# miha-stopar/Plonky3-mobile

Hardware: AMD Instinct MI355X
Metric: fib_air proofs/sec (higher is better)
Workload: dtype u32 (BabyBear Montgomery, 31-bit modular)

## Files before the change

plonky3-mobile_amd/csrc/mmcs.hip:

```cpp
#include <algorithm>

#include "common.h"
#include "mmcs.h"
#include "poseidon2.hip.h"
#include "poseidon2_coop.hip.h"
#include "poseidon2_f64.hip.h"
#include "poseidon2_q4.hip.h"
#include "keccak.hip.h"

namespace p3 {

constexpr int MAX_CLASS_MATS = 16;

struct RowSet {
    const uint32_t* ptr[MAX_CLASS_MATS];
    uint32_t width[MAX_CLASS_MATS];
    uint32_t stride[MAX_CLASS_MATS];
    uint32_t count;
    uint32_t total;
};

__device__ __forceinline__ void load_digest(const uint32_t* p, uint32_t* out8) {
    const uint4* q = reinterpret_cast<const uint4*>(p);
    uint4 a = q[0], b = q[1];
// ... 82 lines not shown
        if (act) {
#pragma unroll
            for (int k = 0; k < 8; k++) lds[tid * 8 + k] = s[k];
            store_digest(out + tid * 8, s);
        }
        __syncthreads();
        out += (size_t)half * 8;
    }
}


__global__ void __launch_bounds__(256) leaf_hash_f64_kernel(const uint32_t* mat, uint32_t width, uint64_t n_rows, uint32_t* digests) {
    if (gridDim.x <= 512u) P3_LATENCY_BOUND_KERNEL();
    uint64_t r = (uint64_t)blockIdx.x * blockDim.x + threadIdx.x;
    if (r >= n_rows) return;
    double s[16];
#pragma unroll
    for (int i = 0; i < 16; i++) s[i] = 0.0;
    const uint32_t* row = mat + r * width;
    for (uint32_t k = 0; k < width; k += 8) {
#pragma unroll
        for (int i = 0; i < 8; i++)
            if (k + i < width) s[i] = p2f::load_elem(row[k + i]);
        p2f::permute(s);
        if (k + 8 < width) {
#pragma unroll
            for (int i = 0; i < 16; i++) s[i] = p2f::reduce(s[i]);
        }
    }
    uint32_t d[8];
    const p2f::MagicRegs smk = p2f::magic_regs();
#pragma unroll
    for (int i = 0; i < 8; i++) d[i] = p2f::store_elem(s[i], smk);
    store_digest(digests + r * 8, d);
}
__global__ void __launch_bounds__(256) compress_layer_q4_kernel(const uint32_t* prev, uint32_t* next, uint64_t n_out, uint32_t prio) {
    if (prio) P3_LATENCY_BOUND_KERNEL();
    const uint32_t q = threadIdx.x & 3u;
    const uint64_t i = ((uint64_t)blockIdx.x * blockDim.x + threadIdx.x) >> 2;
    const bool act = i < n_out;
    const p2q::LaneConsts lc = p2q::lane_consts(q);
    double s[4] = {0.0, 0.0, 0.0, 0.0};
    if (act) {
        const uint4 w = *reinterpret_cast<const uint4*>(prev + i * 16 + 4 * q);
        s[0] = p2f::load_elem(w.x); s[1] = p2f::load_elem(w.y); s[2] = p2f::load_elem(w.z); s[3] = p2f::load_elem(w.w);
    }
    p2q::permute(s, lc, q == 0);
    if (act && q < 2) {
        const p2f::MagicRegs smk = p2f::magic_regs();
        *reinterpret_cast<uint4*>(next + i * 8 + 4 * q) =
            make_uint4(p2f::store_elem(s[0], smk), p2f::store_elem(s[1], smk), p2f::store_elem(s[2], smk), p2f::store_elem(s[3], smk));
    }
}
__global__ void __launch_bounds__(256) leaf_hash_q4_kernel(const uint32_t* mat, uint32_t width, uint64_t n_rows, uint32_t* digests, uint32_t prio) {
    if (prio) P3_LATENCY_BOUND_KERNEL();
    const uint32_t q = threadIdx.x & 3u;
    const uint64_t r = ((uint64_t)blockIdx.x * blockDim.x + threadIdx.x) >> 2;
    const bool act = r < n_rows;
    const p2q::LaneConsts lc = p2q::lane_consts(q);
    double s[4] = {0.0, 0.0, 0.0, 0.0};
    const uint32_t* row = mat + (act ? r : 0) * width;
    for (uint32_t k = 0; k < width; k += 8) {
        if (act && q < 2) {
#pragma unroll
            for (uint32_t i = 0; i < 4; i++)
                if (k + 4 * q + i < width) s[i] = p2f::load_elem(row[k + 4 * q + i]);
        }
        p2q::permute(s, lc, q == 0);
        if (k + 8 < width) {
#pragma unroll
            for (int i = 0; i < 4; i++) s[i] = p2f::reduce(s[i]);
        }
    }
    if (act && q < 2) {
        const p2f::MagicRegs smk = p2f::magic_regs();
        *reinterpret_cast<uint4*>(digests + r * 8 + 4 * q) =
            make_uint4(p2f::store_elem(s[0], smk), p2f::store_elem(s[1], smk), p2f::store_elem(s[2], smk), p2f::store_elem(s[3], smk));
    }
}
constexpr uint32_t LEAF_WIDE_CHUNK = 32, LEAF_WIDE_STRIDE = 36;
__global__ void __launch_bounds__(256) leaf_hash_f64_wide_kernel(const uint32_t* mat, uint32_t width, uint64_t n_rows, uint32_t* digests) {
    __shared__ __attribute__((aligned(16))) uint32_t tile[256 * LEAF_WIDE_STRIDE];
    const uint32_t tid = threadIdx.x, col = tid & 31u, rsub = tid >> 5;
    const uint64_t r0 = (uint64_t)blockIdx.x * 256u, r = r0 + tid;
    double s[16];
#pragma unroll
    for (int i = 0; i < 16; i++) s[i] = 0.0;
    uint32_t pre[32];
    auto fetch = [&](uint32_t c0) {
#pragma unroll
        for (uint32_t i = 0; i < 32; i++) {
            const uint64_t row = r0 + rsub + 8u * i;
            pre[i] = (row < n_rows && c0 + col < width) ? mat[row * width + c0 + col] : 0u;
        }
    };
    fetch(0);
    for (uint32_t c0 = 0; c0 < width; c0 += LEAF_WIDE_CHUNK) {
        __syncthreads();
#pragma unroll
        for (uint32_t i = 0; i < 32; i++) tile[(rsub + 8u * i) * LEAF_WIDE_STRIDE + col] = pre[i];
        __syncthreads();
        if (c0 + LEAF_WIDE_CHUNK < width) fetch(c0 + LEAF_WIDE_CHUNK);
        const uint4* mine = reinterpret_cast<const uint4*>(tile + tid * LEAF_WIDE_STRIDE);
#pragma unroll 1
        for (uint32_t k = 0; k < LEAF_WIDE_CHUNK && c0 + k < width; k += 8) {
            const uint4 a = mine[k / 4], b = mine[k / 4 + 1];
            const uint32_t w[8] = {a.x, a.y, a.z, a.w, b.x, b.y, b.z, b.w};
#pragma unroll
            for (int i = 0; i < 8; i++)
                if (c0 + k + i < width) s[i] = p2f::load_elem(w[i]);
            p2f::permute(s);
            if (c0 + k + 8 < width) {
#pragma unroll
                for (int i = 0; i < 16; i++) s[i] = p2f::reduce(s[i]);
            }
        }
    }
    if (r >= n_rows) return;
    uint32_t d[8];
    const p2f::MagicRegs smk = p2f::magic_regs();
#pragma unroll
    for (int i = 0; i < 8; i++) d[i] = p2f::store_elem(s[i], smk);
    store_digest(digests + r * 8, d);
}
__global__ void __launch_bounds__(256) leaf_hash_f64_rowset_kernel(RowSet rs, uint64_t n_rows, uint32_t* digests) {
    if (gridDim.x <= 512u) P3_LATENCY_BOUND_KERNEL();
    uint64_t r = (uint64_t)blockIdx.x * blockDim.x + threadIdx.x;
    if (r >= n_rows) return;
    double s[16];
#pragma unroll
    for (int i = 0; i < 16; i++) s[i] = 0.0;
    uint32_t m = 0, off = 0;
    for (uint32_t k = 0; k < rs.total; k += 8) {
#pragma unroll
        for (int i = 0; i < 8; i++) {
            if (k + i < rs.total) {
                while (off >= rs.width[m]) { m++; off = 0; }
                s[i] = p2f::load_elem(rs.ptr[m][r * rs.stride[m] + off]);
                off++;
            }
        }
        p2f::permute(s);
        if (k + 8 < rs.total) {
#pragma unroll
            for (int i = 0; i < 16; i++) s[i] = p2f::reduce(s[i]);
        }
    }
    uint32_t d[8];
    const p2f::MagicRegs smk = p2f::magic_regs();
#pragma unroll
    for (int i = 0; i < 8; i++) d[i] = p2f::store_elem(s[i], smk);
    store_digest(digests + r * 8, d);
}
__global__ void __launch_bounds__(256) compress_layer_f64_kernel(const uint32_t* prev, uint32_t* next, uint64_t n_out) {
    if (gridDim.x <= 512u) P3_LATENCY_BOUND_KERNEL();
    uint64_t i = (uint64_t)blockIdx.x * blockDim.x + threadIdx.x;
    if (i >= n_out) return;
    uint32_t w[16];
    load_digest(prev + i * 16, w);
    load_digest(prev + i * 16 + 8, w + 8);
    double s[16];
#pragma unroll
    for (int k = 0; k < 16; k++) s[k] = p2f::load_elem(w[k]);
    p2f::permute(s);
    uint32_t d[8];
    const p2f::MagicRegs smk = p2f::magic_regs();
#pragma unroll
    for (int k = 0; k < 8; k++) d[k] = p2f::store_elem(s[k], smk);
    store_digest(next + i * 8, d);
}

__global__ void __launch_bounds__(256) compress_coop_kernel(const uint32_t* prev, uint32_t* next, uint32_t n_out) {
    P3_LATENCY_BOUND_KERNEL();
    const uint32_t lane16 = threadIdx.x & 15;
    const p2c::LaneConst lc = p2c::lane_constants(lane16);
    uint32_t i = (blockIdx.x * blockDim.x + threadIdx.x) >> 4;
    bool act = i < n_out;
    uint32_t v = act ? prev[(size_t)i * 16 + lane16] : 0u;
    v = p2c::permute(v, lc);
    if (act && lane16 < 8) next[(size_t)i * 8 + lane16] = v;
}
__global__ void __launch_bounds__(256) leaf_coop_kernel(const uint32_t* mat, uint32_t width, uint32_t n_rows, uint32_t* digests) {
    P3_LATENCY_BOUND_KERNEL();
    const uint32_t lane16 = threadIdx.x & 15;
    const p2c::LaneConst lc = p2c::lane_constants(lane16);
    uint32_t r = (blockIdx.x * blockDim.x + threadIdx.x) >> 4;
    bool act = r < n_rows;
    uint32_t v = 0;
    for (uint32_t k = 0; k < width; k += 8) {
        if (act && lane16 < 8 && k + lane16 < width) v = mat[(size_t)r * width + k + lane16];
        v = p2c::permute(v, lc);
    }
    if (act && lane16 < 8) digests[(size_t)r * 8 + lane16] = v;
}
__global__ void __launch_bounds__(1024) tree_levels_coop_kernel(uint32_t* layer_in, uint32_t n_in, uint32_t chunk, uint32_t levels,
                                                                uint32_t* root_copy) {
    P3_LATENCY_BOUND_KERNEL();
    __shared__ uint32_t lds[128 * 8];
    const uint32_t tid = threadIdx.x, lane16 = tid & 15, grp = tid >> 4;
    const p2c::LaneConst lc = p2c::lane_constants(lane16);
    const uint32_t* src = layer_in + (size_t)blockIdx.x * chunk * 8;
    for (uint32_t i = tid; i < chunk * 8; i += blockDim.x) lds[i] = src[i];
    __syncthreads();
    uint32_t* out = layer_in + (size_t)n_in * 8;
    uint32_t cur_n = n_in;
    for (uint32_t l = 0; l < levels; l++) {
        const uint32_t half = chunk >> (l + 1);
        const bool wave_active = ((tid >> 6) << 2) < half;
        uint32_t res = 0;
        if (wave_active) {
            uint32_t v = grp < half ? lds[grp * 16 + lane16] : 0u;
            res = p2c::permute(v, lc);
        }
        __syncthreads();
        if (grp < half && lane16 < 8) {
            lds[grp * 8 + lane16] = res;
            out[((size_t)blockIdx.x * half + grp) * 8 + lane16] = res;
            if (cur_n == 2 && root_copy) root_copy[lane16] = res;
        }
        __syncthreads();
        cur_n >>= 1;
        out += (size_t)cur_n * 8;
    }
}

__global__ void poseidon2_permute_kernel(uint32_t* states, uint64_t n) {
    uint64_t i = (uint64_t)blockIdx.x * blockDim.x + threadIdx.x;
    if (i >= n) return;
    uint32_t s[16];
    uint4* q = reinterpret_cast<uint4*>(states + i * 16);
#pragma unroll
    for (int k = 0; k < 4; k++) { uint4 v = q[k]; s[4 * k] = v.x; s[4 * k + 1] = v.y; s[4 * k + 2] = v.z; s[4 * k + 3] = v.w; }
    p2::permute(s);
#pragma unroll
    for (int k = 0; k < 4; k++) q[k] = make_uint4(s[4 * k], s[4 * k + 1], s[4 * k + 2], s[4 * k + 3]);
}


__global__ void poseidon2_permute_f64_kernel(uint32_t* states, uint64_t n) {
    uint64_t i = (uint64_t)blockIdx.x * blockDim.x + threadIdx.x;
    if (i >= n) return;
    double s[16];
    uint4* q = reinterpret_cast<uint4*>(states + i * 16);
#pragma unroll
    for (int k = 0; k < 4; k++) {
        uint4 v = q[k];
        s[4 * k] = p2f::load_elem(v.x); s[4 * k + 1] = p2f::load_elem(v.y); s[4 * k + 2] = p2f::load_elem(v.z); s[4 * k + 3] = p2f::load_elem(v.w);
    }
    p2f::permute(s);
#pragma unroll
    for (int k = 0; k < 4; k++)
        q[k] = make_uint4(p2f::store_elem(s[4 * k]), p2f::store_elem(s[4 * k + 1]), p2f::store_elem(s[4 * k + 2]), p2f::store_elem(s[4 * k + 3]));
}

__global__ void poseidon2_f64_probe_kernel(const double* in, uint32_t* out, uint64_t n, int mode) {
    uint64_t i = (uint64_t)blockIdx.x * blockDim.x + threadIdx.x;
    if (i >= n) return;
    double s[16];
#pragma unroll
    for (int k = 0; k < 16; k++) s[k] = in[i * 16 + k];
    if (mode == 0) p2f::permute(s);
    else if (mode == 1) p2f::internal_rounds(s, p2f::magic_regs());
    else {
#pragma unroll
        for (int k = 0; k < 16; k++) s[k] = p2f::reduce(s[k]);
    }
#pragma unroll
    for (int k = 0; k < 16; k++) out[i * 16 + k] = p2f::store_elem(s[k]);
}
__global__ void __launch_bounds__(256) poseidon2_q4_probe_kernel(const double* in, uint32_t* out, uint64_t n) {
    const uint32_t q = threadIdx.x & 3u;
    const uint64_t i = ((uint64_t)blockIdx.x * blockDim.x + threadIdx.x) >> 2;
    const bool act = i < n;
    const p2q::LaneConsts lc = p2q::lane_consts(q);
    double s[4] = {0.0, 0.0, 0.0, 0.0};
    if (act) {
#pragma unroll
        for (int k = 0; k < 4; k++) s[k] = in[i * 16 + 4 * q + k];
    }
    p2q::permute(s, lc, q == 0);
    if (act) {
#pragma unroll
        for (int k = 0; k < 4; k++) out[i * 16 + 4 * q + k] = p2f::store_elem(s[k]);
    }
}
int poseidon2_f64_probe(hipStream_t stream, const double* d_in, uint32_t* d_out, uint64_t n, int mode) {
    if (!n) return OK;
    if (mode == 3) hipLaunchKernelGGL(poseidon2_q4_probe_kernel, dim3((uint32_t)((n * 4 + 255) / 256)), dim3(256), 0, stream, d_in, d_out, n);
    else hipLaunchKernelGGL(poseidon2_f64_probe_kernel, dim3((uint32_t)((n + 255) / 256)), dim3(256), 0, stream, d_in, d_out, n, mode);
    P3_HIP(hipGetLastError());
    return OK;
}
__global__ void __launch_bounds__(256) poseidon2_permute_q4_kernel(uint32_t* states, uint64_t n) {
    const uint32_t q = threadIdx.x & 3u;
    const uint64_t i = ((uint64_t)blockIdx.x * blockDim.x + threadIdx.x) >> 2;
    const bool act = i < n;
    const p2q::LaneConsts lc = p2q::lane_consts(q);
    double s[4] = {0.0, 0.0, 0.0, 0.0};
    uint4* mine = reinterpret_cast<uint4*>(states + (act ? i : 0) * 16 + 4 * q);
    if (act) {
        const uint4 w = *mine;
        s[0] = p2f::load_elem(w.x); s[1] = p2f::load_elem(w.y); s[2] = p2f::load_elem(w.z); s[3] = p2f::load_elem(w.w);
    }
    p2q::permute(s, lc, q == 0);
    if (act) {
        const p2f::MagicRegs smk = p2f::magic_regs();
        *mine = make_uint4(p2f::store_elem(s[0], smk), p2f::store_elem(s[1], smk), p2f::store_elem(s[2], smk), p2f::store_elem(s[3], smk));
    }
}
__global__ void __launch_bounds__(256) poseidon2_permute_coop_kernel(uint32_t* states, uint64_t n) {
    const uint32_t lane16 = threadIdx.x & 15;
    const p2c::LaneConst lc = p2c::lane_constants(lane16);
    const uint64_t i = ((uint64_t)blockIdx.x * blockDim.x + threadIdx.x) >> 4;
    const bool act = i < n;
    uint32_t v = act ? states[i * 16 + lane16] : 0u;
    v = p2c::permute(v, lc);
    if (act) states[i * 16 + lane16] = v;
}
int poseidon2_permute_states_variant(hipStream_t stream, uint32_t* d_states, uint64_t n, int variant) {
    if (!n) return OK;
    if (variant == 3) hipLaunchKernelGGL(poseidon2_permute_coop_kernel, dim3((uint32_t)((n * 16 + 255) / 256)), dim3(256), 0, stream, d_states, n);
    else if (variant == 2) hipLaunchKernelGGL(poseidon2_permute_q4_kernel, dim3((uint32_t)((n * 4 + 255) / 256)), dim3(256), 0, stream, d_states, n);
    else if (variant == 1) hipLaunchKernelGGL(poseidon2_permute_f64_kernel, dim3((uint32_t)((n + 255) / 256)), dim3(256), 0, stream, d_states, n);
    else hipLaunchKernelGGL(poseidon2_permute_kernel, dim3((uint32_t)((n + 255) / 256)), dim3(256), 0, stream, d_states, n);
    P3_HIP(hipGetLastError());
    return OK;
}

int poseidon2_permute_states(hipStream_t stream, uint32_t* d_states, uint64_t n) {
    return poseidon2_permute_states_variant(stream, d_states, n, 1);
}

__device__ __forceinline__ uint32_t rowset_elem(const RowSet& rs, uint64_t r, uint32_t k, uint32_t& m, uint32_t& base) {
    while (k - base >= rs.width[m]) { base += rs.width[m]; m++; }
    return rs.ptr[m][r * rs.stride[m] + (k - base)];
}
__device__ __forceinline__ void keccak_sponge_row(const RowSet& rs, uint64_t r, uint64_t (&st)[25]) {
#pragma unroll
    for (int i = 0; i < 25; i++) st[i] = 0;
    const uint32_t n = rs.total, n64 = (n + 1) / 2;
    uint32_t m = 0, base = 0;
    for (uint32_t i = 0; i < n64; i += 17) {
#pragma unroll
        for (int k = 0; k < 17; k++) {
            const uint32_t e = 2 * (i + k);
            if (e < n) {
                uint64_t lo = rowset_elem(rs, r, e, m, base);
                uint64_t hi = e + 1 < n ? rowset_elem(rs, r, e + 1, m, base) : 0u;
                st[k] = lo | (hi << 32);
            }
        }
        if (i + 17 >= n64) kk::permute_digest(st);
        else kk::permute(st);
    }
}
__device__ __forceinline__ void store_digest64(uint32_t* p, const uint64_t (&st)[25]) {
    uint4* q = reinterpret_cast<uint4*>(p);
    q[0] = make_uint4((uint32_t)st[0], (uint32_t)(st[0] >> 32), (uint32_t)st[1], (uint32_t)(st[1] >> 32));
    q[1] = make_uint4((uint32_t)st[2], (uint32_t)(st[2] >> 32), (uint32_t)st[3], (uint32_t)(st[3] >> 32));
}
__global__ void __launch_bounds__(256) keccak_leaf_kernel(RowSet rs, uint64_t n_rows, uint32_t* digests) {
    if (gridDim.x <= 512u) P3_LATENCY_BOUND_KERNEL();
    uint64_t r = (uint64_t)blockIdx.x * blockDim.x + threadIdx.x;
    if (r >= n_rows) return;
    uint64_t st[25];
    keccak_sponge_row(rs, r, st);
    store_digest64(digests + r * 8, st);
}
template <int NP>
struct SaltedRows {
    const uint32_t* mat[NP];
    const uint32_t* salt[NP];
    uint32_t stride;
};
template <int W, int NP>
__global__ void __launch_bounds__(256) keccak_leaf_salted_kernel(SaltedRows<NP> a, uint64_t n_rows, uint32_t* digests) {
    static_assert((W == 4 || W == 6 || W == 8) && NP * (W + 4) <= 34, "one rate block");
    if (gridDim.x <= 512u) P3_LATENCY_BOUND_KERNEL();
    const uint64_t r = (uint64_t)blockIdx.x * blockDim.x + threadIdx.x;
    if (r >= n_rows) return;
    uint64_t st[25];
#pragma unroll
    for (int i = 0; i < 25; i++) st[i] = 0;
#pragma unroll
    for (int p = 0; p < NP; p++) {
        constexpr int L = (W + 4) / 2;
        const uint32_t* m = a.mat[p] + r * a.stride;
        if constexpr (W == 6) {
            const uint2* q = reinterpret_cast<const uint2*>(m);
#pragma unroll
            for (int k = 0; k < 3; k++) { const uint2 v = q[k]; st[p * L + k] = (uint64_t)v.x | ((uint64_t)v.y << 32); }
        } else {
// ... 539 lines not shown
```

plonky3-mobile_amd/csrc/poseidon2_f64.hip.h:

```cpp
#pragma once
#include "poseidon2.hip.h"

namespace p2f {

constexpr double PD = 2013265921.0;
constexpr double PINV = 1.0 / 2013265921.0;

__device__ __forceinline__ double mulmod(double a, double b) {
    double h = a * b;
    double l = __fma_rn(a, b, -h);
    double q = __builtin_rint(h * PINV);
    double r = __fma_rn(-q, PD, h);
    return r + l;
}
constexpr double PM1 = 2013265920.0;
__device__ __forceinline__ double mulmod_p(double a, double b, double aP) {
    double q = __builtin_rint(b * aP);
    double t = __fma_rn(a, b, -(q * PM1));
    return t - q;
}
__device__ __forceinline__ double reduce(double x) {
    return __fma_rn(-__builtin_rint(x * PINV), PD, x);
}
__device__ __forceinline__ double add_scaled_pow2(double tot, double x, double inv) {
    double xt = __fma_rn(x, inv, tot);
    double fr = __builtin_amdgcn_fract(xt);
    return __fma_rn(fr, -PD, xt);
}
constexpr double MAGIC = 6755399441055744.0;
constexpr double MAGIC_P = 6755399441055744.0 * 2013265921.0;
struct MagicRegs { double m, mp; };
__device__ __forceinline__ MagicRegs magic_regs() {
    MagicRegs r{MAGIC, MAGIC_P};
    asm volatile("" : "+v"(r.m), "+v"(r.mp));
    return r;
}
__device__ __forceinline__ double mulmod_m(double a, double b, double aP, const MagicRegs& k, double neg_pm1) {
    const double qb = __fma_rn(b, aP, k.m);
    const double c = __fma_rn(qb, neg_pm1, k.mp);
    const double t = __fma_rn(a, b, c);
    return t - qb;
}
__device__ __forceinline__ double sbox7(double x, const MagicRegs& k, double neg_pm1, double pinv) {
    const double xP = x * pinv;
    const double x2 = mulmod_m(x, x, xP, k, neg_pm1), x3 = mulmod_m(x, x2, xP, k, neg_pm1), x4 = mulmod_m(x, x3, xP, k, neg_pm1);
    return mulmod_m(x3, x4, x3 * pinv, k, neg_pm1);
}

struct ConstsF64 {
    double ext[8][16];
    double in[13];
    double k3, k15, i4, i8, i16, i256;
    double neg_pm1, pinv;
};
constexpr uint32_t c_from_monty(uint32_t m) {
    uint32_t t = m * bb::MU;
    uint64_t u = (uint64_t)t * bb::P;
    uint32_t uh = (uint32_t)(u >> 32);
    return uh ? bb::P - uh : 0;
}
constexpr uint64_t c_powmod(uint64_t b, uint64_t e) { uint64_t r = 1; b %= bb::P; while (e) { if (e & 1) r = r * b % bb::P; b = b * b % bb::P; e >>= 1; } return r; }
constexpr ConstsF64 make_consts() {
    ConstsF64 c{};
    for (int r = 0; r < 4; r++)
        for (int i = 0; i < 16; i++) {
            c.ext[r][i] = (double)c_from_monty(P3_RC16_EXT_INIT_MONTY[r][i]);
            c.ext[4 + r][i] = (double)c_from_monty(P3_RC16_EXT_FINAL_MONTY[r][i]);
        }
    for (int r = 0; r < 13; r++) c.in[r] = (double)c_from_monty(P3_RC16_INTERNAL_MONTY[r]);
    c.k3 = 3.0; c.k15 = 15.0; c.i4 = 0.25; c.i8 = 0.125; c.i16 = 0.0625; c.i256 = 0.00390625;
    c.neg_pm1 = -2013265920.0; c.pinv = 1.0 / 2013265921.0;
    return c;
}
static __device__ __constant__ ConstsF64 d_c = make_consts();

__device__ __forceinline__ void mat4(double& a, double& b, double& c, double& d) {
    double t01 = a + b, t23 = c + d, t0123 = t01 + t23;
    double t01123 = t0123 + b, t01233 = t0123 + d;
    double nd = __fma_rn(a, 2.0, t01233), nb = __fma_rn(c, 2.0, t01123);
    double na = t01123 + t01, nc = t01233 + t23;
    a = na; b = nb; c = nc; d = nd;
}
__device__ __forceinline__ void external_linear(double (&s)[16]) {
#pragma unroll
    for (int i = 0; i < 16; i += 4) mat4(s[i], s[i + 1], s[i + 2], s[i + 3]);
    double t[4];
#pragma unroll
    for (int k = 0; k < 4; k++) t[k] = (s[k] + s[k + 4]) + (s[k + 8] + s[k + 12]);
#pragma unroll
    for (int i = 0; i < 16; i++) s[i] += t[i & 3];
}

__device__ __forceinline__ void internal_rounds(double (&s)[16], const MagicRegs& mk) {
    const double npm1 = d_c.neg_pm1, pinv = d_c.pinv;
    const double k3 = d_c.k3, k15 = d_c.k15, i4 = d_c.i4, i8 = d_c.i8, i16 = d_c.i16, i256 = d_c.i256;
    auto internal_round = [&](int r) {
        s[0] = sbox7(s[0] + d_c.in[r], mk, npm1, pinv);
        double tot = ((s[0] + s[1]) + (s[2] + s[3])) + ((s[4] + s[5]) + (s[6] + s[7])) +
                     (((s[8] + s[9]) + (s[10] + s[11])) + ((s[12] + s[13]) + (s[14] + s[15])));
        tot = reduce(tot);
        s[0] = __fma_rn(s[0], -2.0, tot);
        s[1] = tot + s[1];
        s[2] = __fma_rn(s[2], 2.0, tot);
        s[3] = add_scaled_pow2(tot, s[3], 0.5);
        s[4] = __fma_rn(s[4], k3, tot);
        s[5] = __fma_rn(s[5], 4.0, tot);
        s[6] = add_scaled_pow2(tot, s[6], -0.5);
        s[7] = __fma_rn(s[7], -k3, tot);
        s[8] = __fma_rn(s[8], -4.0, tot);
        s[9] = add_scaled_pow2(tot, s[9], i256);
        s[10] = add_scaled_pow2(tot, s[10], i4);
        s[11] = add_scaled_pow2(tot, s[11], i8);
        s[12] = __fma_rn(s[12], -k15, tot);
        s[13] = add_scaled_pow2(tot, s[13], -i256);
        s[14] = add_scaled_pow2(tot, s[14], -i16);
        s[15] = __fma_rn(s[15], k15, tot);
    };
    auto fold_integer_lanes = [&]() {
        s[1] = reduce(s[1]); s[2] = reduce(s[2]); s[4] = reduce(s[4]); s[5] = reduce(s[5]);
        s[7] = reduce(s[7]); s[8] = reduce(s[8]); s[12] = reduce(s[12]); s[15] = reduce(s[15]);
    };
    _Pragma("clang loop unroll(disable)")
    for (int blk = 0; blk < 3; blk++) {
        _Pragma("clang loop unroll(disable)")
        for (int r = 0; r < 4; r++) internal_round(4 * blk + r);
        fold_integer_lanes();
    }
    internal_round(12);
    fold_integer_lanes();
}

__device__ __forceinline__ void permute(double (&s)[16]) {
    const MagicRegs mk = magic_regs();
    const double npm1 = d_c.neg_pm1, pinv = d_c.pinv;
    external_linear(s);
    _Pragma("clang loop unroll(disable)")
    for (int r = 0; r < 4; r++) {
#pragma unroll
        for (int i = 0; i < 16; i++) s[i] = sbox7(s[i] + d_c.ext[r][i], mk, npm1, pinv);
        external_linear(s);
    }
    internal_rounds(s, mk);
    _Pragma("clang loop unroll(disable)")
    for (int r = 4; r < 8; r++) {
#pragma unroll
        for (int i = 0; i < 16; i++) s[i] = sbox7(s[i] + d_c.ext[r][i], mk, npm1, pinv);
        external_linear(s);
    }
}

__device__ __forceinline__ double load_elem(uint32_t monty) { return (double)bb::from_monty(monty); }
constexpr double R_MOD_P = 268435454.0;
constexpr double R_MOD_P_OVER_P = 268435454.0 / 2013265921.0;
__device__ __forceinline__ uint32_t store_elem(double v, const MagicRegs& k) {
    const double r = mulmod_m(R_MOD_P, v, R_MOD_P_OVER_P, k, d_c.neg_pm1);
    const uint32_t w = (uint32_t)(int32_t)r;
    return min(w, w + bb::P);
}
__device__ __forceinline__ uint32_t store_elem(double v) { return store_elem(v, magic_regs()); }

}
```

plonky3-mobile_amd/csrc/prover.hip:

```cpp
#include <chrono>
#include <cstddef>
#include <deque>
#include <memory>
#include <cstring>

#include "bb31.hip.h"
#include "challenger.h"
#include "common.h"
#include "keccak.hip.h"
#include "mmcs.h"
#include "poseidon2.hip.h"
#include "poseidon2_f64.hip.h"
#include "prover.h"
#include "rng.h"
#include "rng_dev.hip.h"
#include "transcript.hip.h"

namespace p3 {

using bb::Ext;

__device__ __forceinline__ uint32_t tl(const TwoLevelTable& t, uint32_t e) {
    return bb::mul(t.lo[e & ((1u << t.T) - 1u)], t.hi[e >> t.T]);
}
// ... 70 lines not shown
    const DenConsts k0 = ds->k0, k1 = ds->k1;
    uint32_t t = blockIdx.x * blockDim.x + threadIdx.x;
    uint32_t j0 = t * DEN_CHUNK;
    if (j0 >= big) return;
    uint32_t a0[2 * DEN_CHUNK], e0[2 * DEN_CHUNK], e1[2 * DEN_CHUNK], nrm[2 * DEN_CHUNK], pre[2 * DEN_CHUNK];
#pragma unroll
    for (int k = 0; k < DEN_CHUNK; k++) {
        uint32_t x = bb::mul(gen, tl(roots, brev((j0 + k) & (big - 1), log_big)));
#pragma unroll
        for (int z = 0; z < 2; z++) {
            const DenConsts& c = z ? k1 : k0;
            const uint32_t a = bb::sub(c.z0, x);
            const uint32_t dd0 = bb::add(bb::sqr(a), c.k0), dd1 = bb::sub(bb::mul(c.k1, a), c.c1);
            a0[2 * k + z] = a; e0[2 * k + z] = dd0; e1[2 * k + z] = dd1;
            nrm[2 * k + z] = bb::sub(bb::sqr(dd0), bb::mul(bb::W_MONTY, bb::sqr(dd1)));
        }
    }
    uint32_t acc = bb::ONE;
#pragma unroll
    for (int k = 0; k < 2 * DEN_CHUNK; k++) { pre[k] = acc; acc = bb::mul(acc, nrm[k]); }
    uint32_t inv = bb::inv(acc);
#pragma unroll
    for (int k = 2 * DEN_CHUNK - 1; k >= 0; k--) {
        const uint32_t r = bb::mul(inv, pre[k]);
        inv = bb::mul(inv, nrm[k]);
        nrm[k] = r;
    }
#pragma unroll
    for (int k = 0; k < DEN_CHUNK; k++) {
        if (j0 + k >= big) break;
#pragma unroll
        for (int z = 0; z < 2; z++) {
            const DenConsts& c = z ? k1 : k0;
            const uint32_t i = 2 * k + z;
            const uint32_t f0 = bb::mul(e0[i], nrm[i]), f1 = bb::neg(bb::mul(e1[i], nrm[i]));
            Ext r;
            r.c[0] = bb::add(bb::mul(a0[i], f0), bb::mul(c.z2w, f1));
            r.c[2] = bb::add(bb::mul(a0[i], f1), bb::mul(c.z2, f0));
            r.c[1] = bb::neg(bb::add(bb::mul(c.z1, f0), bb::mul(c.z3w, f1)));
            r.c[3] = bb::neg(bb::add(bb::mul(c.z1, f1), bb::mul(c.z3, f0)));
            st_ext((z ? d1 : d0) + 4 * (size_t)(j0 + k), r);
        }
    }
}

constexpr int BARY_BLOCK = 256;
__global__ void __launch_bounds__(BARY_BLOCK) barycentric_kernel(TwoLevelTable roots, uint32_t n, uint32_t log_big,
                                                                 uint32_t gen, const uint2* lde_t, const uint4* lde_q,
                                                                 const uint32_t* d0, const uint32_t* d1,
                                                                 uint32_t* partials) {
    Ext acc[8];
#pragma unroll
    for (int k = 0; k < 8; k++) acc[k] = bb::ext_zero();
    const uint32_t step = gridDim.x * blockDim.x;
    for (uint32_t j = blockIdx.x * blockDim.x + threadIdx.x; j < n; j += 2 * step) {
        const bool two = j + step < n;
        const uint32_t j2 = two ? j + step : j;
        const uint32_t xa = bb::mul(gen, tl(roots, brev(j, log_big))), xb = two ? bb::mul(gen, tl(roots, brev(j2, log_big))) : 0u;
        const Ext e0a = bb::scale(ld_ext(d0 + 4 * (size_t)j), xa), e1a = bb::scale(ld_ext(d1 + 4 * (size_t)j), xa);
        const Ext e0b = bb::scale(ld_ext(d0 + 4 * (size_t)j2), xb), e1b = bb::scale(ld_ext(d1 + 4 * (size_t)j2), xb);
        const uint2 ta = lde_t[j], tb = lde_t[j2];
        const uint4 qa = lde_q[j], qb = lde_q[j2];
        auto fma2 = [](Ext& s, const Ext& ea, uint32_t va, const Ext& eb, uint32_t vb) {
#pragma unroll
            for (int c = 0; c < 4; c++) s.c[c] = bb::add(s.c[c], bb::dot2(ea.c[c], va, eb.c[c], vb));
        };
        fma2(acc[0], e0a, ta.x, e0b, tb.x);
        fma2(acc[1], e0a, ta.y, e0b, tb.y);
        fma2(acc[2], e1a, ta.x, e1b, tb.x);
        fma2(acc[3], e1a, ta.y, e1b, tb.y);
        fma2(acc[4], e0a, qa.x, e0b, qb.x);
        fma2(acc[5], e0a, qa.y, e0b, qb.y);
        fma2(acc[6], e0a, qa.z, e0b, qb.z);
        fma2(acc[7], e0a, qa.w, e0b, qb.w);
    }
    __shared__ uint32_t red[BARY_BLOCK / 64][32];
    const uint32_t lane = threadIdx.x & 63, wave = threadIdx.x >> 6;
#pragma unroll
    for (int k = 0; k < 8; k++)
#pragma unroll
        for (int c = 0; c < 4; c++) {
            uint32_t v = acc[k].c[c];
#pragma unroll
            for (int off = 32; off > 0; off >>= 1) v = bb::add(v, (uint32_t)__shfl_down((int)v, off, 64));
            if (lane == 0) red[wave][4 * k + c] = v;
        }
    __syncthreads();
    if (threadIdx.x < 32) {
        uint32_t v = 0;
#pragma unroll
        for (int w = 0; w < BARY_BLOCK / 64; w++) v = bb::add(v, red[w][threadIdx.x]);
        partials[blockIdx.x * 32 + threadIdx.x] = v;
    }
}

struct ReducedArgs {
    const uint2* lde_t;
    const uint4* lde_q;
    const uint32_t* d0;
    const uint32_t* d1;
    uint32_t* ro;
    const DevState* ds;
    uint32_t big;
};
__global__ void __launch_bounds__(256) reduced_openings_kernel(ReducedArgs a) {
    uint32_t j = blockIdx.x * blockDim.x + threadIdx.x;
    if (j >= a.big) return;
    const DevState* __restrict__ ds = a.ds;
    uint2 t = a.lde_t[j];
    uint4 q = a.lde_q[j];
    Ext u, w;
#pragma unroll
    for (int c = 0; c < 4; c++) {
        u.c[c] = bb::add(bb::add(bb::dot2(ds->alp[4].c[c], q.x, ds->alp[5].c[c], q.y), bb::dot2(ds->alp[6].c[c], q.z, ds->alp[7].c[c], q.w)),
                         bb::mul(ds->alp[1].c[c], t.y));
        w.c[c] = bb::dot2(ds->alp[2].c[c], t.x, ds->alp[3].c[c], t.y);
    }
    u.c[0] = bb::add(u.c[0], t.x);
    Ext e0 = ld_ext(a.d0 + 4 * (size_t)j), e1 = ld_ext(a.d1 + 4 * (size_t)j);
    Ext r = bb::add(bb::mul(bb::sub(ds->y02, u), e0), bb::mul(bb::sub(ds->y1, w), e1));
    st_ext(a.ro + 4 * (size_t)j, r);
}

__global__ void __launch_bounds__(256) fri_fold_kernel(TwoLevelTable inv_roots , const uint32_t* in,
                                                       uint32_t* out, uint32_t half, uint32_t log_half,
                                                       const DevState* __restrict__ ds, uint32_t round, uint32_t one_half) {
    if (gridDim.x <= 512u) P3_LATENCY_BOUND_KERNEL();
    uint32_t i = blockIdx.x * blockDim.x + threadIdx.x;
    if (i >= half) return;
    const Ext half_beta = ds->half_beta[round];
    Ext lo = ld_ext(in + 8 * (size_t)i), hi = ld_ext(in + 8 * (size_t)i + 4);
    uint32_t p = tl(inv_roots, brev(i, log_half));
    Ext s = bb::scale(bb::add(lo, hi), one_half);
    Ext d = bb::mul(bb::scale(half_beta, p), bb::sub(lo, hi));
    st_ext(out + 4 * (size_t)i, bb::add(s, d));
}

__global__ void __launch_bounds__(256) fri_fold_rollin_kernel(TwoLevelTable inv_roots , const uint32_t* in,
                                                              const uint32_t* __restrict__ ro, uint32_t* out, uint32_t half,
                                                              uint32_t log_half, const DevState* __restrict__ ds, uint32_t round,
                                                              uint32_t one_half) {
    if (gridDim.x <= 512u) P3_LATENCY_BOUND_KERNEL();
    uint32_t i = blockIdx.x * blockDim.x + threadIdx.x;
    if (i >= half) return;
    const Ext half_beta = ds->half_beta[round];
    const Ext beta2 = bb::sqr(bb::add(half_beta, half_beta));
    Ext lo = ld_ext(in + 8 * (size_t)i), hi = ld_ext(in + 8 * (size_t)i + 4), e = ld_ext(ro + 4 * (size_t)i);
    uint32_t p = tl(inv_roots, brev(i, log_half));
    Ext s = bb::scale(bb::add(lo, hi), one_half);
    Ext d = bb::mul(bb::scale(half_beta, p), bb::sub(lo, hi));
    st_ext(out + 4 * (size_t)i, bb::add(bb::add(s, d), bb::mul(beta2, e)));
}

__global__ void __launch_bounds__(256) grind_kernel(DevState* ds, uint32_t mask, uint32_t base) {
    uint32_t w = base + blockIdx.x * blockDim.x + threadIdx.x;
    if (w >= bb::P) return;
    if (base + blockIdx.x * blockDim.x > *(volatile uint32_t*)&ds->grind_result) return;
    const uint32_t pos = ds->n_in;
    double s[16];
#pragma unroll
    for (int i = 0; i < 16; i++) s[i] = p2f::load_elem((i < 8 && (uint32_t)i < pos) ? ds->inb[i & 7] : ds->st[i]);
#pragma unroll
    for (int i = 0; i < 8; i++) s[i] = (i == (int)pos) ? (double)w : s[i];
    p2f::permute(s);
    if ((bb::from_monty(p2f::store_elem(s[7])) & mask) == 0) atomicMin(&ds->grind_result, w);
}

__global__ void __launch_bounds__(256) grind_keccak_kernel(DevState* ds, uint32_t mask, uint32_t base) {
    uint32_t w = base + blockIdx.x * blockDim.x + threadIdx.x;
    if (w >= bb::P) return;
    if (base + blockIdx.x * blockDim.x > *(volatile uint32_t*)&ds->grind_result) return;
    const KeccakGrindArgs& a = ds->kgrind;
    const uint32_t wm = bb::to_monty(w);
    uint64_t st[25];
#pragma unroll
    for (int i = 0; i < 25; i++) st[i] = a.state[i];
    for (uint32_t blk = 0; blk < a.n_blocks; blk++) {
#pragma unroll
        for (int i = 0; i < 17; i++) {
            uint64_t lane = a.block[blk][i];
            const int32_t rel = (int32_t)(a.wpos) - (int32_t)(blk * 136 + i * 8);
            if (rel > -4 && rel < 8) {
                const uint64_t v = (uint64_t)wm;
                lane ^= rel >= 0 ? (v << (8 * rel)) : (v >> (8 * -rel));
            }
            st[i] ^= lane;
        }
        if (blk + 1 == a.n_blocks) kk::permute_digest(st);
        else kk::permute(st);
    }
    bool ok = false;
#pragma unroll
    for (int t = 0; t < 8; t++) {
        const uint64_t lane = st[3 - t / 2];
        const uint32_t hi_or_lo = (t & 1) ? (uint32_t)lane : (uint32_t)(lane >> 32);
        const uint32_t v = __builtin_bswap32(hi_or_lo) & 0x7fffffffu;
        if (v < bb::P) { ok = (v & mask) == 0; break; }
    }
    if (ok) atomicMin(&ds->grind_result, w);
}

constexpr uint32_t QTREE_MAX_MATS = 8;
struct QTree {
    const uint32_t* mat[QTREE_MAX_MATS];
    uint32_t width[QTREE_MAX_MATS];
    uint32_t stride[QTREE_MAX_MATS];
    uint32_t n_mats;
    const uint32_t* layers;
    uint32_t log_height, shift, slot_off;
    uint32_t mshift[QTREE_MAX_MATS];
};
__global__ void query_gather_kernel(const QTree* trees, const uint32_t* indices, uint32_t slot_words, uint32_t* out) {
    P3_LATENCY_BOUND_KERNEL();
    const QTree& t = trees[blockIdx.y];
    const uint64_t index = (indices[blockIdx.x] >> t.shift) & ((1ull << t.log_height) - 1ull);
    uint32_t* dst = out + (size_t)blockIdx.x * slot_words + t.slot_off;
    uint32_t off = 0;
    for (uint32_t m = 0; m < t.n_mats; m++) {
        const uint64_t row = index >> t.mshift[m];
        for (uint32_t c = threadIdx.x; c < t.width[m]; c += blockDim.x) dst[off + c] = t.mat[m][row * t.stride[m] + c];
        off += t.width[m];
    }
    uint64_t base = 0, len = 1ull << t.log_height;
    for (uint32_t i = 0; i < t.log_height; i++) {
        const uint64_t sib = (index >> i) ^ 1;
        if (threadIdx.x < 8) dst[off + i * 8 + threadIdx.x] = t.layers[base + sib * 8 + threadIdx.x];
        base += len * 8;
        len >>= 1;
    }
}

struct StageLayout {
    uint32_t root_t = 0, root_q = 8, opened = 16, froots = 48, fpoly = 0, witness = 0, status = 0, qidx = 0, slots = 0, words = 0;
};
struct TsArgs {
    DevState* ds;
    uint32_t* ps;
    int kind;
    StageLayout lay;
};
struct TsPis {
    uint32_t w[3];
    uint32_t given;
};

__global__ void __launch_bounds__(64) ts_begin_kernel(TsArgs a, const uint32_t* trace, uint32_t n, uint32_t log_n, TsPis given) {
    P3_LATENCY_BOUND_KERNEL();
    __shared__ KState ks;
    DevChal ch;
    ch.begin(a.kind, a.ds, &ks, true);
    uint32_t pis[3];
    if (given.given) {
        for (int k = 0; k < 3; k++) pis[k] = given.w[k];
    } else {
        pis[0] = trace[0]; pis[1] = trace[1]; pis[2] = trace[2 * (size_t)(n - 1) + 1];
    }
    ch.observe(bb::to_monty(log_n));
    ch.observe(bb::to_monty(log_n));
    ch.observe_n(a.ps + a.lay.root_t, 8);
    ch.observe_n(pis, 3);
    const Ext alpha = ch.sample_ext();
    Ext ap[5];
    ap[0] = bb::ext_one();
#pragma unroll
    for (int k = 1; k < 5; k++) ap[k] = bb::mul(ap[k - 1], alpha);
    if (threadIdx.x == 0) {
        for (int k = 0; k < 3; k++) a.ds->pis[k] = pis[k];
        for (int k = 0; k < 5; k++) a.ds->apow[k] = ap[k];
        a.ds->status = 0;
        a.ps[a.lay.status] = 0;
    }
    ch.end();
}
__global__ void __launch_bounds__(64) ts_zeta_kernel(TsArgs a, uint32_t g_n) {
    P3_LATENCY_BOUND_KERNEL();
    __shared__ KState ks;
    DevChal ch;
    ch.begin(a.kind, a.ds, &ks, false);
    ch.observe_n(a.ps + a.lay.root_q, 8);
    const Ext zeta = ch.sample_ext();
    const Ext zeta_next = bb::scale(zeta, g_n);
    if (threadIdx.x == 0) {
        a.ds->zeta = zeta;
        a.ds->zeta_next = zeta_next;
        a.ds->k0 = den_consts(zeta);
        a.ds->k1 = den_consts(zeta_next);
    }
    ch.end();
}
constexpr int TS_OPEN_THREADS = 256;
__global__ void __launch_bounds__(TS_OPEN_THREADS) ts_open_kernel(TsArgs a, const uint32_t* partials, uint32_t n_blocks,
                                                                  uint32_t log_n, uint32_t sn, uint32_t denom) {
    P3_LATENCY_BOUND_KERNEL();
    __shared__ KState ks;
    __shared__ uint32_t red[TS_OPEN_THREADS / 32][32];
    __shared__ uint32_t tot[32];
    {
        const uint32_t col = threadIdx.x & 31u, part = threadIdx.x >> 5;
        uint32_t v = 0;
        constexpr uint32_t STEP = TS_OPEN_THREADS / 32;
        uint32_t b = part;
        for (; b + 3 * STEP < n_blocks; b += 4 * STEP) {
            const uint32_t p0 = partials[b * 32 + col], p1 = partials[(b + STEP) * 32 + col],
                           p2 = partials[(b + 2 * STEP) * 32 + col], p3 = partials[(b + 3 * STEP) * 32 + col];
            v = bb::add(bb::add(v, bb::add(p0, p1)), bb::add(p2, p3));
        }
        for (; b < n_blocks; b += STEP) v = bb::add(v, partials[b * 32 + col]);
// ... 723 lines not shown
```

Baseline: 559.3.

## Defer dyadic-lane reductions in Poseidon2 f64 internal rounds and raise occupancy bounds

Replaces the per-round fract-based reduction of each fractionally scaled lane with plain FMAs. Each lane is now folded only when its accumulated fractional bits would exceed a 16-bit budget, using a constexpr schedule, and the internal-round loop is fully unrolled. Integer lanes get their own fold schedules, and the total splits integer and fractional lanes so only one fold is needed. Several f64 Poseidon2 kernels also get __launch_bounds__(256, 8) to push occupancy, at the risk of register spills and of precision errors if the fold schedule is wrong.

After: 573.2, median of 6. 1.02x the previous value.

```diff
diff --git a/plonky3-mobile_amd/csrc/mmcs.hip b/plonky3-mobile_amd/csrc/mmcs.hip
--- a/plonky3-mobile_amd/csrc/mmcs.hip
+++ b/plonky3-mobile_amd/csrc/mmcs.hip
@@ -258,7 +258,7 @@
     for (int i = 0; i < 8; i++) d[i] = p2f::store_elem(s[i], smk);
     store_digest(digests + r * 8, d);
 }
-__global__ void __launch_bounds__(256) compress_layer_f64_kernel(const uint32_t* prev, uint32_t* next, uint64_t n_out) {
+__global__ void __launch_bounds__(256, 8) compress_layer_f64_kernel(const uint32_t* prev, uint32_t* next, uint64_t n_out) {
     if (gridDim.x <= 512u) P3_LATENCY_BOUND_KERNEL();
     uint64_t i = (uint64_t)blockIdx.x * blockDim.x + threadIdx.x;
     if (i >= n_out) return;
@@ -343,7 +343,7 @@
 }
 
 
-__global__ void poseidon2_permute_f64_kernel(uint32_t* states, uint64_t n) {
+__global__ void __launch_bounds__(256, 8) poseidon2_permute_f64_kernel(uint32_t* states, uint64_t n) {
     uint64_t i = (uint64_t)blockIdx.x * blockDim.x + threadIdx.x;
     if (i >= n) return;
     double s[16];
diff --git a/plonky3-mobile_amd/csrc/poseidon2_f64.hip.h b/plonky3-mobile_amd/csrc/poseidon2_f64.hip.h
--- a/plonky3-mobile_amd/csrc/poseidon2_f64.hip.h
+++ b/plonky3-mobile_amd/csrc/poseidon2_f64.hip.h
@@ -91,43 +91,58 @@
     for (int i = 0; i < 16; i++) s[i] += t[i & 3];
 }
 
+__device__ __forceinline__ double fold_dyadic(double x) {
+    return __fma_rn(__builtin_amdgcn_fract(x), -PD, x);
+}
+
+constexpr int FRAC_BUDGET = 16;
+constexpr uint32_t dyadic_fold_rounds(int k) {
+    uint32_t m = 0;
+    for (int r = 0, f = 0; r < 13; r++) {
+        f += k;
+        if (f + k > FRAC_BUDGET || r == 12) { m |= 1u << r; f = 0; }
+    }
+    return m;
+}
+constexpr uint32_t FOLD_K1 = dyadic_fold_rounds(1), FOLD_K2 = dyadic_fold_rounds(2), FOLD_K3 = dyadic_fold_rounds(3),
+                   FOLD_K4 = dyadic_fold_rounds(4), FOLD_K8 = dyadic_fold_rounds(8);
+constexpr uint32_t FOLD_X2 = 1u << 12, FOLD_X4 = (1u << 6) | (1u << 12), FOLD_X15 = (1u << 3) | (1u << 7) | (1u << 12);
+static_assert(FOLD_K1 == 0x1000 && FOLD_K2 == 0x1080 && FOLD_K3 == 0x1210 && FOLD_K4 == 0x1888 && FOLD_K8 == 0x1aaa, "fold schedule");
 __device__ __forceinline__ void internal_rounds(double (&s)[16], const MagicRegs& mk) {
     const double npm1 = d_c.neg_pm1, pinv = d_c.pinv;
     const double k3 = d_c.k3, k15 = d_c.k15, i4 = d_c.i4, i8 = d_c.i8, i16 = d_c.i16, i256 = d_c.i256;
     auto internal_round = [&](int r) {
         s[0] = sbox7(s[0] + d_c.in[r], mk, npm1, pinv);
-        double tot = ((s[0] + s[1]) + (s[2] + s[3])) + ((s[4] + s[5]) + (s[6] + s[7])) +
-                     (((s[8] + s[9]) + (s[10] + s[11])) + ((s[12] + s[13]) + (s[14] + s[15])));
-        tot = reduce(tot);
+        const double ti = (((s[0] + s[1]) + (s[2] + s[4])) + ((s[5] + s[7]) + (s[8] + s[12]))) + s[15];
+        const double tf = ((s[3] + s[6]) + (s[9] + s[10])) + ((s[11] + s[13]) + s[14]);
+        const double tot = reduce(ti + fold_dyadic(tf));
         s[0] = __fma_rn(s[0], -2.0, tot);
         s[1] = tot + s[1];
         s[2] = __fma_rn(s[2], 2.0, tot);
-        s[3] = add_scaled_pow2(tot, s[3], 0.5);
+        s[3] = __fma_rn(s[3], 0.5, tot);
         s[4] = __fma_rn(s[4], k3, tot);
         s[5] = __fma_rn(s[5], 4.0, tot);
-        s[6] = add_scaled_pow2(tot, s[6], -0.5);
+        s[6] = __fma_rn(s[6], -0.5, tot);
         s[7] = __fma_rn(s[7], -k3, tot);
         s[8] = __fma_rn(s[8], -4.0, tot);
-        s[9] = add_scaled_pow2(tot, s[9], i256);
-        s[10] = add_scaled_pow2(tot, s[10], i4);
-        s[11] = add_scaled_pow2(tot, s[11], i8);
+        s[9] = __fma_rn(s[9], i256, tot);
+        s[10] = __fma_rn(s[10], i4, tot);
+        s[11] = __fma_rn(s[11], i8, tot);
         s[12] = __fma_rn(s[12], -k15, tot);
-        s[13] = add_scaled_pow2(tot, s[13], -i256);
-        s[14] = add_scaled_pow2(tot, s[14], -i16);
+        s[13] = __fma_rn(s[13], -i256, tot);
+        s[14] = __fma_rn(s[14], -i16, tot);
         s[15] = __fma_rn(s[15], k15, tot);
+        if (FOLD_K1 >> r & 1) { s[3] = fold_dyadic(s[3]); s[6] = fold_dyadic(s[6]); }
+        if (FOLD_K8 >> r & 1) { s[9] = fold_dyadic(s[9]); s[13] = fold_dyadic(s[13]); }
+        if (FOLD_K2 >> r & 1) s[10] = fold_dyadic(s[10]);
+        if (FOLD_K3 >> r & 1) s[11] = fold_dyadic(s[11]);
+        if (FOLD_K4 >> r & 1) s[14] = fold_dyadic(s[14]);
+        if (FOLD_X2 >> r & 1) { s[1] = reduce(s[1]); s[2] = reduce(s[2]); }
+        if (FOLD_X4 >> r & 1) { s[4] = reduce(s[4]); s[5] = reduce(s[5]); s[7] = reduce(s[7]); s[8] = reduce(s[8]); }
+        if (FOLD_X15 >> r & 1) { s[12] = reduce(s[12]); s[15] = reduce(s[15]); }
     };
-    auto fold_integer_lanes = [&]() {
-        s[1] = reduce(s[1]); s[2] = reduce(s[2]); s[4] = reduce(s[4]); s[5] = reduce(s[5]);
-        s[7] = reduce(s[7]); s[8] = reduce(s[8]); s[12] = reduce(s[12]); s[15] = reduce(s[15]);
-    };
-    _Pragma("clang loop unroll(disable)")
-    for (int blk = 0; blk < 3; blk++) {
-        _Pragma("clang loop unroll(disable)")
-        for (int r = 0; r < 4; r++) internal_round(4 * blk + r);
-        fold_integer_lanes();
-    }
-    internal_round(12);
-    fold_integer_lanes();
+#pragma unroll
+    for (int r = 0; r < 13; r++) internal_round(r);
 }
 
 __device__ __forceinline__ void permute(double (&s)[16]) {
diff --git a/plonky3-mobile_amd/csrc/prover.hip b/plonky3-mobile_amd/csrc/prover.hip
--- a/plonky3-mobile_amd/csrc/prover.hip
+++ b/plonky3-mobile_amd/csrc/prover.hip
@@ -246,7 +246,7 @@
     st_ext(out + 4 * (size_t)i, bb::add(bb::add(s, d), bb::mul(beta2, e)));
 }
 
-__global__ void __launch_bounds__(256) grind_kernel(DevState* ds, uint32_t mask, uint32_t base) {
+__global__ void __launch_bounds__(256, 8) grind_kernel(DevState* ds, uint32_t mask, uint32_t base) {
     uint32_t w = base + blockIdx.x * blockDim.x + threadIdx.x;
     if (w >= bb::P) return;
     if (base + blockIdx.x * blockDim.x > *(volatile uint32_t*)&ds->grind_result) return;
```
